# NVIDIA/audio-flamingo

Measured on AMD Instinct MI355X. Metric: audio-sec/s + decoder tokens/s, AF3-7B bf16 train, higher is better.
Workload: dtype bf16; 1 GPU; AF3 (AF-Whisper 32L + Qwen2.5-7B 28L, MLP projector) bf16 train step fwd+bwd+AdamW, 30 s clips, S=1024; micro_batch_per_gpu=8, global_batch=8, seq_len=1024, parallelism=dp1, activation_checkpointing=False

## Files before the change

audio-flamingo_amd/csrc/common.h:

```cpp
#pragma once
#include <hip/hip_runtime.h>
#include <stdint.h>
#include <stdio.h>
#include <stdarg.h>
#include <type_traits>
#include <utility>

typedef __bf16 bf16;
typedef __attribute__((ext_vector_type(2))) __bf16 bf16x2;
typedef __attribute__((ext_vector_type(4))) __bf16 bf16x4;
typedef __attribute__((ext_vector_type(8))) __bf16 bf16x8;
typedef __attribute__((ext_vector_type(2))) float f32x2;
typedef __attribute__((ext_vector_type(4))) float f32x4;
typedef __attribute__((ext_vector_type(16))) float f32x16;

#define AFK_OK 0
#define AFK_ERR_ARG (-1)
#define AFK_ERR_LAUNCH (-2)
#define AFK_ERR_UNSUPPORTED (-3)

int afk_set_error(int code, const char* fmt, ...);
void afk_count(int id);

#define AFK_REQUIRE(cond, ...)                                   \
// ... 110 lines not shown
    for (int i = 0; i < NW; ++i) r += scratch[i];
    return r;
}
template <int NW>
__device__ __forceinline__ float block_max(float v, float* scratch) {
    v = wave_max(v);
    const int lane = threadIdx.x & 63, w = threadIdx.x >> 6;
    __syncthreads();
    if (lane == 0) scratch[w] = v;
    __syncthreads();
    float r = scratch[0];
#pragma unroll
    for (int i = 1; i < NW; ++i) r = fmaxf(r, scratch[i]);
    return r;
}

__device__ __forceinline__ float sigmoid_f(float x) { return 1.f / (1.f + __expf(-x)); }
__device__ __forceinline__ float gelu_f(float x) { return 0.5f * x * (1.f + erff(x * 0.70710678118654752440f)); }
__device__ __forceinline__ float gelu_grad_f(float x) {
    const float cdf = 0.5f * (1.f + erff(x * 0.70710678118654752440f));
    const float pdf = 0.39894228040143267794f * __expf(-0.5f * x * x);
    return cdf + x * pdf;
}
```

audio-flamingo_amd/csrc/elementwise.hip:

```cpp
#include "common.h"
#include "../../include/afk.h"

namespace {

inline int ew_grid(int64_t n_items, int per_block) {
    int64_t g = afk_cdiv(n_items, per_block);
    if (g > 4096) g = 4096;
    if (g < 1) g = 1;
    return (int)g;
}

__global__ __launch_bounds__(256) void transpose_kernel(const bf16* __restrict__ in0, bf16* __restrict__ out0, int R, int C,
                                                        int Rpad, int64_t ld_in, int64_t ld_out, int nb2,
                                                        int64_t bs1_in, int64_t bs2_in, int64_t bs1_out, int64_t bs2_out,
                                                        int tiles_x, int tiles_y, int64_t ntiles) {
    __shared__ bf16 tile[64][66];
    const int t = threadIdx.x;
    for (int64_t tix = blockIdx.x; tix < ntiles; tix += gridDim.x) {
        const int bx = (int)(tix % tiles_x);
        const int by = (int)((tix / tiles_x) % tiles_y);
        const int b = (int)(tix / ((int64_t)tiles_x * tiles_y));
        const int b1 = b / nb2, b2 = b - b1 * nb2;
        const bf16* in = in0 + b1 * bs1_in + b2 * bs2_in;
        bf16* out = out0 + b1 * bs1_out + b2 * bs2_out;
        const int r0 = by * 64, c0 = bx * 64;
#pragma unroll
        for (int k = 0; k < 2; ++k) {
            const int idx = t + 256 * k;
            const int r = idx >> 3, ch = idx & 7;
            const int gr = r0 + r, gc = c0 + ch * 8;
            bf16x8 v;
            if (gr < R && gc + 7 < C) {
                v = *(const bf16x8*)(in + (int64_t)gr * ld_in + gc);
// ... 17 lines not shown
                if (gr + 7 < Rpad) {
                    *(bf16x8*)(out + (int64_t)gc * ld_out + gr) = v;
                } else {
                    for (int e = 0; e < 8 && gr + e < Rpad; ++e) out[(int64_t)gc * ld_out + gr + e] = v[e];
                }
            }
        }
        __syncthreads();
    }
}

__global__ __launch_bounds__(256) void gelu_bwd_kernel(const bf16* __restrict__ dy, const bf16* __restrict__ pre,
                                                       bf16* __restrict__ dx, int64_t nvec) {
    for (int64_t i = (int64_t)blockIdx.x * 256 + threadIdx.x; i < nvec; i += (int64_t)gridDim.x * 256) {
        const bf16x8 d = *(const bf16x8*)(dy + 8 * i);
        const bf16x8 p = *(const bf16x8*)(pre + 8 * i);
        bf16x8 o;
#pragma unroll
        for (int e = 0; e < 8; ++e) o[e] = (bf16)((float)d[e] * gelu_grad_f((float)p[e]));
        *(bf16x8*)(dx + 8 * i) = o;
    }
}

__global__ __launch_bounds__(256) void gelu_fwd_kernel(const bf16* __restrict__ x, bf16* __restrict__ y, int64_t nvec) {
    for (int64_t i = (int64_t)blockIdx.x * 256 + threadIdx.x; i < nvec; i += (int64_t)gridDim.x * 256) {
        const bf16x8 p = *(const bf16x8*)(x + 8 * i);
        bf16x8 o;
#pragma unroll
        for (int e = 0; e < 8; ++e) o[e] = (bf16)gelu_f((float)p[e]);
        *(bf16x8*)(y + 8 * i) = o;
    }
}


__global__ __launch_bounds__(256) void silu_mul_fwd_kernel(const bf16* __restrict__ gu, bf16* __restrict__ h, int64_t rows,
                                                           int I) {
    const int vpr = I >> 3;
    const int64_t total = rows * vpr;
    for (int64_t i = (int64_t)blockIdx.x * 256 + threadIdx.x; i < total; i += (int64_t)gridDim.x * 256) {
        const int64_t r = i / vpr;
        const int c = (int)(i - r * vpr) * 8;
        const bf16x8 g = *(const bf16x8*)(gu + r * 2 * I + c);
        const bf16x8 u = *(const bf16x8*)(gu + r * 2 * I + I + c);
        bf16x8 o;
#pragma unroll
        for (int e = 0; e < 8; ++e) {
            const float gf = (float)g[e];
            o[e] = (bf16)(rbf(gf * sigmoid_f(gf)) * (float)u[e]);
        }
        *(bf16x8*)(h + r * I + c) = o;
    }
}
// ... 683 lines not shown

#define ST ((hipStream_t)stream)

extern "C" int afk_transpose_bf16(const void* in, void* out, int R, int C, int Rpad, int64_t ld_in, int64_t ld_out, int nb1,
                                  int nb2, int64_t bs1_in, int64_t bs2_in, int64_t bs1_out, int64_t bs2_out, int max_blocks,
                                  void* stream) {
    AFK_REQUIRE(in && out && R > 0 && C > 0 && Rpad >= R && nb1 > 0 && nb2 > 0, "afk_transpose_bf16: bad args");
    AFK_REQUIRE(ld_in % 8 == 0 && ld_out % 8 == 0 && ((uintptr_t)in % 16 == 0) && ((uintptr_t)out % 16 == 0) &&
                    bs1_in % 8 == 0 && bs2_in % 8 == 0 && bs1_out % 8 == 0 && bs2_out % 8 == 0,
                "afk_transpose_bf16: 16-byte alignment required");
    const int tiles_x = (int)afk_cdiv(C, 64), tiles_y = (int)afk_cdiv(Rpad, 64);
    const int64_t ntiles = (int64_t)tiles_x * tiles_y * nb1 * nb2;
    int64_t grid = ntiles;
    if (grid > 65536) grid = 65536;
    if (max_blocks > 0 && grid > max_blocks) grid = max_blocks;
    hipLaunchKernelGGL(transpose_kernel, dim3((unsigned)grid), dim3(256), 0, ST, (const bf16*)in, (bf16*)out, R, C, Rpad, ld_in, ld_out,
                       nb2, bs1_in, bs2_in, bs1_out, bs2_out, tiles_x, tiles_y, ntiles);
    AFK_LAUNCH_CHECK("afk_transpose_bf16");
    return AFK_OK;
}

extern "C" int afk_gelu_fwd(const void* x, void* y, int64_t n, void* stream) {
    AFK_REQUIRE(x && y && n % 8 == 0, "afk_gelu_fwd: n must be a multiple of 8");
    hipLaunchKernelGGL(gelu_fwd_kernel, dim3(ew_grid(n / 8, 256)), dim3(256), 0, ST, (const bf16*)x, (bf16*)y, n / 8);
    AFK_LAUNCH_CHECK("afk_gelu_fwd");
    return AFK_OK;
}

extern "C" int afk_gelu_bwd(const void* dy, const void* pre, void* dx, int64_t n, void* stream) {
    AFK_REQUIRE(dy && pre && dx && n % 8 == 0, "afk_gelu_bwd: n must be a multiple of 8");
    hipLaunchKernelGGL(gelu_bwd_kernel, dim3(ew_grid(n / 8, 256)), dim3(256), 0, ST, (const bf16*)dy, (const bf16*)pre,
                       (bf16*)dx, n / 8);
    AFK_LAUNCH_CHECK("afk_gelu_bwd");
    return AFK_OK;
}

extern "C" int afk_silu_mul_fwd(const void* gu, void* h, int64_t rows, int I, void* stream) {
    AFK_REQUIRE(gu && h && I % 8 == 0 && rows > 0, "afk_silu_mul_fwd: bad args");
    hipLaunchKernelGGL(silu_mul_fwd_kernel, dim3(ew_grid(rows * (I / 8), 256)), dim3(256), 0, ST, (const bf16*)gu, (bf16*)h,
                       rows, I);
    AFK_LAUNCH_CHECK("afk_silu_mul_fwd");
    return AFK_OK;
}

extern "C" int afk_silu_mul_bwd(const void* gu, const void* dh, void* dgu, int64_t rows, int I, void* stream) {
    AFK_REQUIRE(gu && dh && dgu && I % 8 == 0 && rows > 0, "afk_silu_mul_bwd: bad args");
    hipLaunchKernelGGL(silu_mul_bwd_kernel, dim3(ew_grid(rows * (I / 8), 256)), dim3(256), 0, ST, (const bf16*)gu,
// ... 398 lines not shown
```

audio-flamingo_amd/csrc/gemm.hip:

```cpp
#include "gemm_common.h"
#include <vector>
#include <mutex>

namespace {

constexpr int BM = 128, BN = 128, BK = 64;
constexpr int ROWB = BK * 2;
constexpr int STAGE_BYTES = (BM + BN) * ROWB;
constexpr int NSTAGE = 2;

__global__ __launch_bounds__(256, 2) void gemm_nt_bf16_k128(GemmArgs p) {
    extern __shared__ __attribute__((aligned(16))) char smem[];
    const int tid = threadIdx.x;
    const int lane = tid & 63;
    const int wave = __builtin_amdgcn_readfirstlane(tid >> 6);
    const int wm = wave >> 1, wn = wave & 1;
    const int hi = lane >> 5, l31 = lane & 31;

    int tm, tn;
    gemm_tile_of_block(p, tm, tn);
    const int m0 = tm * BM, n0 = tn * BN;

    const bf16* a_src[4];
    const bf16* b_src[4];
// ... 314 lines not shown
        if (flags & (AFK_GEMM_RESIDUAL | AFK_GEMM_SWIGLU_BWD)) w = w && ldr % 8 == 0 && (uintptr_t)residual % 16 == 0;
        if (preact_out) w = w && (uintptr_t)preact_out % 16 == 0;
        p.wide = w && g_wide ? 1 : 0;
    }
    const int64_t tiles256 = afk_cdiv(M, 256) * afk_cdiv(N, 256);
    const bool use256 = !gemv && (trans_b || (flags & AFK_GEMM_SWIGLU_FWD) || (splits == 1 && (g_variant >= 2 || (g_variant == 0 && tiles256 >= 192))));
    if (rope && (!use256 || !p.wide || trans_a || trans_b || splits != 1))
        return afk_set_error(AFK_ERR_UNSUPPORTED, "afk_gemm_nt_bf16_rope: needs the 256 x 256 NT kernel (>= 192 tiles) in its 16-byte epilogue form; use "
                                                  "afk_gemm_nt_bf16 + afk_rope_inplace for this shape");
#ifdef AFK_PROBES
    static const int env_impl = [] {
        const char* e = getenv("AFK_GEMM256");
        return (e && e[0] == 'p' && e[1] == 'e') ? 13 : (e && e[0] == 'p') ? 2 : (e && e[0] == 'w') ? 3 : (e && e[0] == 'f') ? 10 : 0;
    }();
    const int impl256 = (flags & (AFK_GEMM_SWIGLU_FWD | AFK_GEMM_ROPE)) ? 2 : g_variant >= 2 ? (g_variant == 15 ? 2 : g_variant) : (env_impl ? env_impl : g_256_impl);
    const bool w4 = use256 && !trans_b && impl256 >= 3 && impl256 <= 9;
    const bool f8 = use256 && !trans_b && impl256 >= 10 && impl256 <= 12;
    const bool persist = use256 && !trans_b && impl256 == 13;
    const bool persist_q = use256 && !trans_b && impl256 == 14;
#endif
    if ((flags & AFK_GEMM_SWIGLU_FWD) && !p.wide)
        return afk_set_error(AFK_ERR_UNSUPPORTED, "afk_gemm_nt_bf16: SWIGLU_FWD needs the 16-byte epilogue form (aligned C / preact_out, ldc %% 8 == 0, "
                                                  "afk_gemm_set_variant bit 4 clear)");
    p.ntm = (int)afk_cdiv(M, use256 ? 256 : BM);
    p.ntn = (int)afk_cdiv(N, use256 ? 256 : BN);
    static bool attr_set = false;
    if (!attr_set) {
        hipFuncSetAttribute((const void*)gemm_nt_bf16_k128, hipFuncAttributeMaxDynamicSharedMemorySize, NSTAGE * STAGE_BYTES);
        attr_set = true;
    }
    hipStream_t st = (hipStream_t)stream;
    const int64_t nwg = (int64_t)p.ntm * p.ntn;
    AFK_REQUIRE(nwg < (1ll << 31), "afk_gemm_nt_bf16: grid too large");
    hipEvent_t e0 = nullptr, e1 = nullptr;
    bool prof = false;
    {
        std::lock_guard<std::mutex> lk(g_prof.mu);
        prof = g_prof.on;
        if (prof) {
            e0 = prof_next_event();
            e1 = prof_next_event();
            g_prof.flops += 2.0 * (double)M * (double)N * (double)K;
            g_prof.launches += 1;
            g_prof.recs.push_back({M, N, K, trans_b ? (trans_a ? 4 : 3) : (use256 ? 2 : 1)});
        }
    }
// ... 103 lines not shown
```

audio-flamingo_amd/csrc/gemm256.hip:

```cpp
#include "gemm_common.h"

namespace {

constexpr int BM = 256, BN = 256, BK = 64;
constexpr int ROWB = 128;
constexpr int OP_BYTES = 256 * ROWB;
constexpr int BUF_BYTES = 2 * OP_BYTES;
constexpr int LDS_BYTES = 2 * BUF_BYTES;

#define AFK_VMCNT(n) asm volatile("s_waitcnt vmcnt(" #n ")" ::: "memory")
#define AFK_LGKMCNT0() asm volatile("s_waitcnt lgkmcnt(0)" ::: "memory")
#define AFK_BARRIER()                         \
    do {                                      \
        __builtin_amdgcn_sched_barrier(0);    \
        __builtin_amdgcn_s_barrier();         \
        __builtin_amdgcn_sched_barrier(0);    \
    } while (0)

template <int EPI, int MF, bool OLDLOOP = false>
__global__ __launch_bounds__(512, 1) void gemm_nt_bf16_k256(GemmArgs p) {
    extern __shared__ __attribute__((aligned(16))) char smem[];
    const int tid = threadIdx.x;
    const int lane = tid & 63;
    const int wave = __builtin_amdgcn_readfirstlane(tid >> 6);
    const int wm = wave >> 2, wn = wave & 3;
    const int hi = lane >> 5, l31 = lane & 31;

    int tm, tn;
    gemm_tile_of_block(p, tm, tn);
    const int m0 = tm * BM, n0 = tn * BN;
    const int T = p.K / BK;
// ... 27 lines not shown
            __builtin_amdgcn_global_load_lds((gbl_void*)(xsrc[j] + koff), (lds_void*)(base + xdst[j]), 16, 0, 0);
    };
    auto issue_y = [&](int t) {
        char* base = smem + (t & 1) * BUF_BYTES;
        const int koff = t * BK;
#pragma unroll
        for (int j = 0; j < 2; ++j)
            __builtin_amdgcn_global_load_lds((gbl_void*)(ysrc[j] + koff), (lds_void*)(base + ydst[j]), 16, 0, 0);
    };
    __builtin_amdgcn_sched_barrier(0);
    issue_x(0);
    __builtin_amdgcn_sched_barrier(0);
#pragma unroll
    for (int j = 0; j < 2; ++j) {
        const int jj = wave + 8 * j;
        const int unit = jj < 8 ? 8 + jj : 16 + jj;
        const int rl = unit * 8 + lrow;
        const int chunk = pos ^ ((rl >> 1) & 7);
        const int r = min(m0 + rl, p.M - 1);
        ysrc[j] = p.A + (int64_t)r * p.lda + chunk * 8;
        ydst[j] = unit * 1024;
    }
    issue_y(0);
    if (T > 1) issue_x(1);
    __builtin_amdgcn_sched_barrier(0);

    int koffb[4];
#pragma unroll
    for (int x = 0; x < 4; ++x) koffb[x] = gemm_frag_rowoff<MF>(x) * ROWB + gemm_frag_koff<MF>(x, lane);
    const int a_row0 = (wm * 128 + gemm_frag_row<MF>(lane)) * ROWB;
    const int b_row0 = OP_BYTES + (wn * 64 + gemm_frag_row<MF>(lane)) * ROWB;

    GemmAcc<MF> acc;
    acc.zero();
#pragma unroll
    for (int x = 0; x < 4; ++x) afk_pin(koffb[x]);
    int a_row0_ = a_row0, b_row0_ = b_row0;
    afk_pin(a_row0_);
    afk_pin(b_row0_);
    acc.pin();

    if (T > 1) AFK_VMCNT(8);
    else AFK_VMCNT(2);
    AFK_BARRIER();
    if (wm == 1) AFK_BARRIER();

    bf16x8 bf[2][4], af[2][4];
    auto mfma_group = [&](auto acc0_, auto g_) {
        constexpr int ACC0 = decltype(acc0_)::value, g = decltype(g_)::value;
        if constexpr (MF == 32) {
#pragma unroll
            for (int i = 0; i < 2; ++i)
#pragma unroll
                for (int j = 0; j < 2; ++j) acc.mma(ACC0 + i, j, bf[j][g], af[i][g]);
        } else {
            constexpr int s = g >> 1, i = g & 1;
#pragma unroll
            for (int ih = 0; ih < 2; ++ih)
#pragma unroll
                for (int jt = 0; jt < 4; ++jt) acc.mma(2 * (ACC0 + i) + ih, jt, bf[jt >> 1][2 * (jt & 1) + s], af[i][2 * ih + s]);
        }
    };
    auto mfma_slot = [&](auto acc0_, auto q_) {
        constexpr int ACC0 = decltype(acc0_)::value, q = decltype(q_)::value;
        if constexpr (MF == 32) {
            constexpr int s = q >> 1, i = q & 1;
// ... 179 lines not shown
            const int64_t lbase = lanes ? (((int64_t)((m0 + wm * 128 + i * 32) % p.rope_S) >> 5) * 16 * 32 + l31) * 8 : 0;
#pragma unroll
            for (int j = 0; j < 2; ++j)
#pragma unroll
                for (int t = 0; t < 2; ++t) {
                    const int q = (i * 2 + j) * 2 + t;
                    const int cl = wn * 64 + j * 32 + 16 * t + 8 * hi;
                    b8 o = pc[q];
                    if (rot) {
                        const int d = cl & 127;
                        const b8 other = *(const b8*)(theirs + q * 1024);
                        const b8 c = lanes ? *(const b8*)(p.rope_cos_lanes + lbase + (d >> 3) * 256) : *(const b8*)(p.rope_cos + pr * 128 + d);
                        const b8 sn = lanes ? *(const b8*)(p.rope_sin_lanes + lbase + (d >> 3) * 256) : *(const b8*)(p.rope_sin + pr * 128 + d);
                        const float sg = (wn & 1) ? 1.f : -1.f;
#pragma unroll
                        for (int e = 0; e < 8; ++e)
                            o[e] = (bf16)(rbf_strict((float)pc[q][e] * (float)c[e]) + rbf_strict(sg * (float)other[e] * (float)sn[e]));
                    }
                    if (m < p.M) *(b8*)((bf16*)p.C + (int64_t)m * p.ldc + n0 + cl) = o;
                }
        }
        return;
    }
    if (AFK_GM_NOEPI(p)) return;
#pragma unroll
    for (int i = 0; i < 4; ++i)
#pragma unroll
        for (int j = 0; j < 2; ++j) gemm_store_block32<EPI, MF>(p, m0 + wm * 128 + i * 32, n0 + wn * 64 + j * 32, lane, acc.block(i, j));
}

}

#define AFK_EPI_LIST(X) X(0) X(AFK_GEMM_BIAS) X(AFK_GEMM_RESIDUAL) X(AFK_GEMM_BIAS | AFK_GEMM_RESIDUAL) X(AFK_GEMM_BIAS | AFK_GEMM_GELU) \
    X(AFK_GEMM_BIAS | AFK_GEMM_GELU | AFK_GEMM_RESIDUAL) X(AFK_GEMM_ACCUM) X(AFK_GEMM_SWIGLU_FWD) X(AFK_GEMM_SWIGLU_BWD) X(AFK_GEMM_ROPE) X(AFK_GEMM_ROPE | AFK_GEMM_BIAS) X(-1)

template <int MF, bool OLD = false>
static int launch_gemm256(const GemmArgs& p, hipStream_t st) {
    static bool attr_set = false;
    if (!attr_set) {
#define AFK_SET(F)                                                                                                                           \
    if (hipFuncSetAttribute((const void*)gemm_nt_bf16_k256<(F), MF, OLD>, hipFuncAttributeMaxDynamicSharedMemorySize, LDS_BYTES) != hipSuccess) \
        return afk_set_error(AFK_ERR_LAUNCH, "gemm256: cannot reserve %d bytes of LDS", LDS_BYTES);
        AFK_EPI_LIST(AFK_SET)
#undef AFK_SET
        attr_set = true;
    }
    const int64_t nwg = (int64_t)p.ntm * p.ntn;
    const int f = (p.wide && p.splits <= 1) ? p.flags : -1;
    switch (f) {
#define AFK_CASE(F)                                                                                              \
    case (F):                                                                                                    \
        if ((F) == -1) afk_count(AFK_CNT_GEMM_GENERIC);                                                          \
        hipLaunchKernelGGL((gemm_nt_bf16_k256<(F), MF, OLD>), dim3((unsigned)nwg), dim3(512), LDS_BYTES, st, p);      \
        break;
        AFK_EPI_LIST(AFK_CASE)
#undef AFK_CASE
        default:
            afk_count(AFK_CNT_GEMM_GENERIC);
            hipLaunchKernelGGL((gemm_nt_bf16_k256<-1, MF, OLD>), dim3((unsigned)nwg), dim3(512), LDS_BYTES, st, p);
    }
    return AFK_OK;
}

int afk_launch_gemm256(const GemmArgs& p, int mf, hipStream_t st) {
#ifdef AFK_PROBES
    if (AFK_GM_OLDLOOP(p)) return mf == 16 ? launch_gemm256<16, true>(p, st) : launch_gemm256<32, true>(p, st);
#endif
    if constexpr ((AFK_MFMA_SHAPES_NT & 2) != 0)
        if (mf == 16) return launch_gemm256<16>(p, st);
    if constexpr ((AFK_MFMA_SHAPES_NT & 1) != 0)
        if (mf == 32) return launch_gemm256<32>(p, st);
    return afk_set_error(AFK_ERR_UNSUPPORTED, "gemm256: the %s MFMA shape of the NT kernel is built under make PROBES=1 only", mf == 16 ? "16x16x32" : "32x32x16");
}
```

audio-flamingo_amd/csrc/gemm_common.h:

```cpp
#pragma once
#include "common.h"
#include "../../include/afk.h"

struct GemmArgs {
    const bf16* A;
    const bf16* B;
    void* C;
    void* C2;
    const bf16* bias;
    const bf16* R;
    int64_t lda, ldb, ldc, ldr;
    int M, N, K;
    int ntm, ntn;
    int flags;
    int res_mod;
    float alpha;
    int gm;
    int splits;
    float* ws;
    int wide;
    const bf16* rope_cos;
    const bf16* rope_sin;
    const int* rope_pos;
    int rope_S, rope_cols;
    const bf16* rope_cos_lanes;
    const bf16* rope_sin_lanes;
};

#ifdef AFK_PROBES
#define AFK_GM_NOEPI(p) (((p).gm & 0x40) != 0)
#define AFK_GM_RAW(p) (((p).gm & 0x80) != 0)
#define AFK_GM_OLDLOOP(p) (((p).gm & 0x100) != 0)
#else
#define AFK_GM_NOEPI(p) false
#define AFK_GM_RAW(p) false
#endif

typedef __attribute__((address_space(3))) void lds_void;
typedef const __attribute__((address_space(1))) void gbl_void;

__device__ __forceinline__ void gemm_tile_of(const GemmArgs& p, int bid, int nwg, int& tm, int& tn) {
    const int xcd = bid & 7, idx = bid >> 3, q = nwg >> 3, r = nwg & 7;
    const int swz = AFK_GM_RAW(p) ? bid : (xcd < r ? xcd * (q + 1) : r * (q + 1) + (xcd - r) * q) + idx;
    const int GM = (p.gm & 0x3f) > 0 ? (p.gm & 0x3f) : 4;
    const int per_group = GM * p.ntn;
    const int g = swz / per_group, rem = swz - g * per_group;
    const int first_m = g * GM;
    const int gsz = min(p.ntm - first_m, GM);
    tm = first_m + rem % gsz;
    tn = rem / gsz;
}
__device__ __forceinline__ void gemm_tile_of_block(const GemmArgs& p, int& tm, int& tn) { gemm_tile_of(p, blockIdx.x, gridDim.x, tm, tn); }

template <int W, int F = -1>
__device__ __forceinline__ void gemm_epilogue_store(const GemmArgs& p, int m, int n, float* v) {
    typedef __attribute__((ext_vector_type(W))) __bf16 bvec;
    typedef __attribute__((ext_vector_type(W))) float fvec;
    const int flags = F >= 0 ? F : p.flags;
#pragma unroll
    for (int e = 0; e < W; ++e) v[e] *= p.alpha;
    if (flags & AFK_GEMM_BIAS) {
        const bvec bv = *(const bvec*)(p.bias + n);
#pragma unroll
        for (int e = 0; e < W; ++e) v[e] += (float)bv[e];
    }
    if (flags & AFK_GEMM_GELU) {
#pragma unroll
        for (int e = 0; e < W; ++e) v[e] = rbf(v[e]);
        if (p.C2) {
            bvec pre;
#pragma unroll
            for (int e = 0; e < W; ++e) pre[e] = (bf16)v[e];
            *(bvec*)((bf16*)p.C2 + (int64_t)m * p.ldc + n) = pre;
        }
#pragma unroll
        for (int e = 0; e < W; ++e) v[e] = gelu_f(v[e]);
    }
    if (flags & AFK_GEMM_SWIGLU_BWD) {
        const bvec gv = *(const bvec*)(p.R + (int64_t)m * p.ldr + n);
        const bvec uv = *(const bvec*)(p.R + (int64_t)m * p.ldr + p.N + n);
        bvec og, ou;
#pragma unroll
        for (int e = 0; e < W; ++e) {
            const float gf = (float)gv[e], uf = (float)uv[e], df = rbf(v[e]);
            const float s = sigmoid_f(gf);
            og[e] = (bf16)(df * uf * (s * (1.f + gf * (1.f - s))));
            ou[e] = (bf16)(df * (gf * s));
        }
        bf16* cp = (bf16*)p.C + (int64_t)m * p.ldc + n;
        *(bvec*)cp = og;
        *(bvec*)(cp + p.N) = ou;
        return;
    }
    if (flags & AFK_GEMM_RESIDUAL) {
        const int rm = p.res_mod > 0 ? m % p.res_mod : m;
        const bvec rv = *(const bvec*)(p.R + (int64_t)rm * p.ldr + n);
#pragma unroll
        for (int e = 0; e < W; ++e) v[e] = rbf(v[e]) + (float)rv[e];
    }
// ... 93 lines not shown
__device__ __forceinline__ void gemm_lane_swap(float x, float y, float& lo, float& hi) {
    if constexpr (MF == 16) {
        const auto r = __builtin_amdgcn_permlane16_swap(__float_as_uint(x), __float_as_uint(y), false, false);
        lo = __uint_as_float(r[0]);
        hi = __uint_as_float(r[1]);
    } else {
        const auto r = __builtin_amdgcn_permlane32_swap(__float_as_uint(x), __float_as_uint(y), false, false);
        lo = __uint_as_float(r[0]);
        hi = __uint_as_float(r[1]);
    }
}
template <int MF>
__device__ __forceinline__ void gemm_quad_pos(int lane, int t, int h, int& row, int& col) {
    if (MF == 16) {
        row = 16 * h + (lane & 15);
        col = 16 * t + 4 * (lane >> 4);
    } else {
        row = lane & 31;
        col = 8 * (2 * t + h) + 4 * (lane >> 5);
    }
}

template <int F, int MF>
__device__ __forceinline__ void gemm_store_block32_body(const GemmArgs& p, int mb, int nb, int lane, const f32x16& b);
template <int MF>
static __device__ __noinline__ void gemm_store_block32_generic(const GemmArgs& p, int mb, int nb, int lane, f32x16 b) {
    gemm_store_block32_body<-1, MF>(p, mb, nb, lane, b);
}
template <int F = -1, int MF = 32>
__device__ __forceinline__ void gemm_store_block32(const GemmArgs& p, int mb, int nb, int lane, const f32x16& b) {
    if constexpr (F == -1) gemm_store_block32_generic<MF>(p, mb, nb, lane, b);
    else gemm_store_block32_body<F, MF>(p, mb, nb, lane, b);
}
template <int F, int MF>
__device__ __forceinline__ void gemm_store_block32_body(const GemmArgs& p, int mb, int nb, int lane, const f32x16& b) {
    if (F == -2 || (F == -1 && p.splits > 1)) {
#pragma unroll
        for (int t = 0; t < 2; ++t)
#pragma unroll
            for (int h = 0; h < 2; ++h) {
                int row, col;
                gemm_quad_pos<MF>(lane, t, h, row, col);
                const int m = mb + row, n = nb + col;
                if (m >= p.M || n >= p.N) continue;
                const f32x4 o = {b[8 * t + 4 * h], b[8 * t + 4 * h + 1], b[8 * t + 4 * h + 2], b[8 * t + 4 * h + 3]};
                *(f32x4*)(p.ws + ((int64_t)blockIdx.y * p.M + m) * p.N + n) = o;
            }
        return;
    }
    if constexpr (F == -2) return;
    if (F >= 0 || p.wide) {
        const int m = mb + (lane & 31);
#pragma unroll
        for (int t = 0; t < 2; ++t) {
            float v[8];
#pragma unroll
            for (int e = 0; e < 4; ++e) gemm_lane_swap<MF>(b[8 * t + e], b[8 * t + 4 + e], v[e], v[4 + e]);
            const int n = nb + 16 * t + 8 * (lane >> 5);
            if (m < p.M && n < p.N) gemm_epilogue_store<8, F>(p, m, n, v);
        }
        return;
    }
#pragma unroll
    for (int t = 0; t < 2; ++t)
#pragma unroll
        for (int h = 0; h < 2; ++h) {
            int row, col;
            gemm_quad_pos<MF>(lane, t, h, row, col);
            const int m = mb + row, n = nb + col;
            if (m >= p.M || n >= p.N) continue;
            float v[4] = {b[8 * t + 4 * h], b[8 * t + 4 * h + 1], b[8 * t + 4 * h + 2], b[8 * t + 4 * h + 3]};
            gemm_epilogue_store<4, F>(p, m, n, v);
        }
}

#ifdef AFK_PROBES
#define AFK_MFMA_SHAPES_NT 3
#define AFK_MFMA_SHAPES_NN 3
#define AFK_MFMA_SHAPES_TN 3
#else
#define AFK_MFMA_SHAPES_NT 2
#define AFK_MFMA_SHAPES_NN 1
// ... 10 lines not shown
```

audio-flamingo_amd/csrc/norm.hip:

```cpp
#include <algorithm>
#include "common.h"
#include "../../include/afk.h"

namespace {

constexpr int ROWS_PER_BLOCK = 4;
typedef __attribute__((ext_vector_type(4))) unsigned u32x4;

template <int VPL, bool RMS, int VW>
__global__ __launch_bounds__(256) void norm_fwd_kernel(const bf16* __restrict__ x, const bf16* __restrict__ w,
                                                       const bf16* __restrict__ b, bf16* __restrict__ y,
                                                       float* __restrict__ mean_out, float* __restrict__ rstd_out,
                                                       int64_t rows, int D, float eps) {
    const int lane = threadIdx.x & 63, wv = threadIdx.x >> 6;
    typedef __attribute__((ext_vector_type(VW))) __bf16 bvec;
    const int nvec = D / VW;
    const float invD = 1.f / (float)D;
    for (int64_t row = (int64_t)blockIdx.x * ROWS_PER_BLOCK + wv; row < rows; row += (int64_t)gridDim.x * ROWS_PER_BLOCK) {
        const bf16* xr = x + row * D;
        float v[VPL][VW];
        float s = 0.f, ss = 0.f;
#pragma unroll
        for (int i = 0; i < VPL; ++i) {
            const int vi = lane + 64 * i;
// ... 435 lines not shown
    return AFK_OK;
}

extern "C" int afk_layernorm_bwd(const void* x, const void* w, const void* dy, const float* mean, const float* rstd,
                                 void* dx, const void* dx_add, void* dw, void* db, int accumulate, float* workspace,
                                 int64_t rows, int D, void* stream) {
    AFK_REQUIRE(x && w && dy && mean && rstd && dx && dw && db && workspace, "afk_layernorm_bwd: null pointer");
    AFK_REQUIRE(D % 4 == 0 && D <= 4096 && (D <= 3584 || D % 8 == 0) && rows > 0, "afk_layernorm_bwd: unsupported D=%d", D);
    AFK_NORM_BWD_ALIGN("afk_layernorm_bwd");
    AFK_REQUIRE((uintptr_t)db % 8 == 0, "afk_layernorm_bwd: db must be 8-byte aligned");
    const bool cols = norm_bwd_use_cols(D);
    AFK_REQUIRE(cols || D <= 3584, "afk_layernorm_bwd: D=%d > 3584 is not served by the row-per-wave form (AFK_NORM_BWD=rows)", D);
    const int nb = std::min(cols ? norm_bwd_cols_blocks(rows, D, false) : norm_bwd_rowwave_blocks(rows), afk_norm_bwd_blocks(rows));
    hipStream_t st = (hipStream_t)stream;
    if (cols) launch_bwd_cols<false>(x, w, dy, mean, rstd, dx, dx_add, workspace, nb, rows, D, st);
    else launch_bwd<false>(x, w, dy, mean, rstd, dx, dx_add, workspace, nb, rows, D, st);
    hipLaunchKernelGGL(fold_partials_kernel, dim3((unsigned)afk_cdiv(D, 64), 2), dim3(256), 0, st, workspace, nb, D, 2 * D, (bf16*)dw, (bf16*)db,
                       accumulate);
    AFK_LAUNCH_CHECK("afk_layernorm_bwd");
    return AFK_OK;
}

namespace {
__global__ __launch_bounds__(256) void gelu_bwd_colsum_kernel(const bf16* __restrict__ dy, const bf16* __restrict__ pre, bf16* __restrict__ dx, int64_t rows, int C,
                                                              float* __restrict__ partials) {
    const int col = (blockIdx.y * 256 + threadIdx.x) * 8;
    if (col >= C) return;
    float pc[8];
#pragma unroll
    for (int e = 0; e < 8; ++e) pc[e] = 0.f;
    const int64_t step = gridDim.x;
    int64_t r = blockIdx.x;
    for (; r + 3 * step < rows; r += 4 * step) {
        bf16x8 d[4], p[4];
#pragma unroll
        for (int u = 0; u < 4; ++u) {
            d[u] = *(const bf16x8*)(dy + (r + u * step) * C + col);
            p[u] = *(const bf16x8*)(pre + (r + u * step) * C + col);
        }
#pragma unroll
        for (int u = 0; u < 4; ++u) {
            bf16x8 o;
#pragma unroll
            for (int e = 0; e < 8; ++e) {
                o[e] = (bf16)((float)d[u][e] * gelu_grad_f((float)p[u][e]));
                pc[e] += (float)o[e];
            }
            *(bf16x8*)(dx + (r + u * step) * C + col) = o;
        }
    }
    for (; r < rows; r += step) {
        const bf16x8 d = *(const bf16x8*)(dy + r * C + col), p = *(const bf16x8*)(pre + r * C + col);
        bf16x8 o;
#pragma unroll
        for (int e = 0; e < 8; ++e) {
            o[e] = (bf16)((float)d[e] * gelu_grad_f((float)p[e]));
            pc[e] += (float)o[e];
        }
        *(bf16x8*)(dx + r * C + col) = o;
    }
    float* outp = partials + (int64_t)blockIdx.x * C + col;
    *(f32x4*)(outp) = f32x4{pc[0], pc[1], pc[2], pc[3]};
    *(f32x4*)(outp + 4) = f32x4{pc[4], pc[5], pc[6], pc[7]};
}
}

extern "C" int afk_gelu_bwd_colsum_parts(int64_t rows) {
    static const int cap = [] { const char* e = getenv("AFK_GELU_CS_PARTS"); const int v = e ? atoi(e) : 0; return v > 0 ? v : 512; }();
    return (int)(rows < cap ? (rows < 1 ? 1 : rows) : cap);
}

extern "C" int afk_gelu_bwd_colsum(const void* dy, const void* pre, void* dx, int64_t rows, int C, void* colsum, int colsum_accumulate, float* workspace,
                                   void* stream) {
    AFK_REQUIRE(dy && pre && dx && colsum && workspace && rows > 0 && C > 0 && C % 8 == 0, "afk_gelu_bwd_colsum: bad arguments (C %% 8 == 0)");
    AFK_REQUIRE((uintptr_t)dy % 16 == 0 && (uintptr_t)pre % 16 == 0 && (uintptr_t)dx % 16 == 0 && (uintptr_t)workspace % 16 == 0 && (uintptr_t)colsum % 8 == 0,
                "afk_gelu_bwd_colsum: dy / pre / dx / workspace must be 16-byte aligned, colsum 8-byte aligned");
    hipStream_t st = (hipStream_t)stream;
    const int np = afk_gelu_bwd_colsum_parts(rows);
    hipLaunchKernelGGL(gelu_bwd_colsum_kernel, dim3((unsigned)np, (unsigned)afk_cdiv(C / 8, 256)), dim3(256), 0, st, (const bf16*)dy, (const bf16*)pre, (bf16*)dx, rows, C,
                       workspace);
    hipLaunchKernelGGL(fold_partials_kernel, dim3((unsigned)afk_cdiv(C, 64), 1), dim3(256), 0, st, workspace, np, C, C, (bf16*)colsum, (bf16*)nullptr, colsum_accumulate);
    AFK_LAUNCH_CHECK("afk_gelu_bwd_colsum");
    return AFK_OK;
}

extern "C" int afk_layernorm_bwd_colsum(const void* x, const void* w, const void* dy, const float* mean, const float* rstd, void* dx, const void* dx_add,
                                        void* dw, void* db, int accumulate, void* colsum, int colsum_accumulate, float* workspace, int64_t rows, int D,
                                        void* stream) {
    AFK_REQUIRE(x && w && dy && mean && rstd && dx && dx_add && dw && db && colsum && workspace, "afk_layernorm_bwd_colsum: null pointer");
    AFK_REQUIRE(D % 8 == 0 && D / 8 <= 512 && rows > 0, "afk_layernorm_bwd_colsum: unsupported D=%d (D %% 8 == 0, D <= 4096)", D);
    AFK_NORM_BWD_ALIGN("afk_layernorm_bwd_colsum");
    AFK_REQUIRE((uintptr_t)db % 8 == 0 && (uintptr_t)colsum % 8 == 0, "afk_layernorm_bwd_colsum: db / colsum must be 8-byte aligned");
    const int nb = std::min(norm_bwd_cols_blocks(rows, D, false), afk_norm_bwd_blocks(rows));
    hipStream_t st = (hipStream_t)stream;
    float* cs = workspace + (int64_t)afk_norm_bwd_blocks(rows) * 2 * D;
    const int nt = (int)afk_cdiv(D / 8, 64) * 64;
    hipLaunchKernelGGL((norm_bwd_cols_kernel<false, true, 2, true>), dim3(nb), dim3(nt), 0, st, (const bf16*)x, (const bf16*)w, (const bf16*)dy, mean, rstd,
                       (bf16*)dx, (const bf16*)dx_add, workspace, rows, D, cs);
    hipLaunchKernelGGL(fold_partials_kernel, dim3((unsigned)afk_cdiv(D, 64), 3), dim3(256), 0, st, workspace, nb, D, 2 * D, (bf16*)dw, (bf16*)db, accumulate,
                       (const float*)cs, D, (bf16*)colsum, colsum_accumulate);
    AFK_LAUNCH_CHECK("afk_layernorm_bwd_colsum");
    return AFK_OK;
}
// ... 19 lines not shown
```

audio-flamingo_amd/ops.py:

```python
from __future__ import annotations

import os

import torch

from . import _lib
from ._lib import AfkError

BF16 = torch.bfloat16

GEMM_BIAS, GEMM_GELU, GEMM_RESIDUAL, GEMM_OUT_F32, GEMM_ACCUM, GEMM_SWIGLU_BWD, GEMM_SWIGLU_FWD = 1, 2, 4, 8, 16, 32, 64


def _stream() -> int:
    return torch.cuda.current_stream().cuda_stream


def _p(t):
    return 0 if t is None else t.data_ptr()


def _chk(t: torch.Tensor, dtype=None, name="tensor"):
    if not t.is_cuda:
        raise AfkError(f"{name}: expected a HIP device tensor, got {t.device} (no CPU fallback in this package)")
# ... 1167 lines not shown
    if ws is None:
        ws = torch.empty(_lib.load().afk_sumsq_workspace_floats(), device=x.device, dtype=torch.float32)
    _lib.call("afk_sumsq_bf16", x.data_ptr(), x.numel(), _chk(acc, torch.float32).data_ptr(), _p(gate), ws.data_ptr(), _stream())
    return acc


def clip_coef_(sumsq, coef, *, max_norm, scale=1.0, norm_out=None):
    _lib.call("afk_clip_coef", _chk(sumsq, torch.float32).data_ptr(), sumsq.numel(), float(scale), float(max_norm), coef.data_ptr(), _p(norm_out), _stream())


def set_f32(dst, values):
    v = [float(x) for x in values] + [0.0] * (4 - len(values))
    _lib.call("afk_set_f32", _chk(dst, torch.float32).data_ptr(), len(values), v[0], v[1], v[2], v[3], _stream())


def gemm_set_variant(v: int):
    _lib.call("afk_gemm_set_variant", int(v))


def gemm_set_mfma(v: int):
    _lib.call("afk_gemm_set_mfma", int(v))


def gemm_mfma_shapes(form: str) -> tuple:
    mask = _lib.load().afk_gemm_mfma_shapes(("nt", "nn", "tn").index(form))
    return tuple(v for v in (1, 2) if mask >> (v - 1) & 1)


KERNEL_FAMILIES = ("gemm_nt128", "gemm_nt256", "gemm_nn256", "gemm_tn256", "gemm_splitk", "gemv", "attn2_fwd_d64", "attn2_fwd_d128",
                   "attn2_bwd_d64", "attn2_bwd_d128", "gqa_reduce", "xattn_fwd", "xattn_bwd", "attn1_fwd", "attn1_bwd", "gemm_generic_epilogue")


def kernel_counts(reset: bool = False) -> dict:
    import ctypes

    buf = (ctypes.c_int64 * len(KERNEL_FAMILIES))()
    _lib.call("afk_kernel_counts", ctypes.addressof(buf), len(KERNEL_FAMILIES))
    if reset:
        _lib.call("afk_kernel_counts_reset")
    return dict(zip(KERNEL_FAMILIES, list(buf)))


def prof_enable(on: bool):
    _lib.call("afk_prof_enable", int(on))


# ... 10 lines not shown
```

include/afk.h:

```cpp
#ifndef AFK_H
#define AFK_H
#include <stdint.h>
#ifdef __cplusplus
extern "C" {
#endif

int afk_version(void);
const char* afk_last_error(void);
const char* afk_build_id(void);
int afk_has_probes(void);

#define AFK_CNT_GEMM_NT128 0
#define AFK_CNT_GEMM_NT256 1
#define AFK_CNT_GEMM_NN256 2
#define AFK_CNT_GEMM_TN256 3
#define AFK_CNT_GEMM_SPLITK 4
#define AFK_CNT_GEMV 5
#define AFK_CNT_ATTN2_FWD_D64 6
#define AFK_CNT_ATTN2_FWD_D128 7
#define AFK_CNT_ATTN2_BWD_D64 8
#define AFK_CNT_ATTN2_BWD_D128 9
#define AFK_CNT_GQA_REDUCE 10
#define AFK_CNT_XATTN_FWD 11
#define AFK_CNT_XATTN_BWD 12
#define AFK_CNT_ATTN1_FWD 13
#define AFK_CNT_ATTN1_BWD 14
#define AFK_CNT_GEMM_GENERIC 15
#define AFK_CNT_MAX 16
int afk_kernel_counts(int64_t* host_out, int n);
int afk_kernel_counts_reset(void);

int afk_prof_enable(int on);
int afk_prof_reset(void);
int afk_prof_collect(double* host_total_ms, double* host_total_flops, int64_t* host_launches);
int afk_prof_dump(const char* host_path);

int afk_gemm_set_variant(int variant);
int afk_gemm_set_mfma(int v);
int afk_gemm_mfma_shapes(int form);
#define AFK_GEMM_BIAS 1
#define AFK_GEMM_GELU 2
#define AFK_GEMM_RESIDUAL 4
#define AFK_GEMM_OUT_F32 8
#define AFK_GEMM_ACCUM 16
#define AFK_GEMM_SWIGLU_BWD 32
#define AFK_GEMM_ROPE 128
#define AFK_GEMM_SWIGLU_FWD 64
int afk_gemm_nt_bf16(const void* A, int64_t lda, const void* B, int64_t ldb, void* C, int64_t ldc,
                     int M, int N, int K, const void* bias, const void* residual, int64_t ldr,
                     int res_mod, void* preact_out, float alpha, int flags, void* stream);
int afk_gemm_bf16(int trans_a, int trans_b, const void* A, int64_t lda, const void* B, int64_t ldb, void* C,
                  int64_t ldc, int M, int N, int K, const void* bias, const void* residual, int64_t ldr,
                  int res_mod, void* preact_out, float alpha, int flags, void* stream);
// ... 326 lines not shown
```

Measured before the change: 642.4 audio-s/s.

## Replace GELU erf evaluation with bf16-indexed LDS lookup tables

Builds per-device lookup tables of GELU and its gradient, indexed by bf16 bit pattern over a window of exponents, and stages them into LDS in the GEMM GELU epilogue, the standalone gelu forward kernel and the gelu backward colsum kernel. Vectors whose inputs all fall inside the window use a table read; the rest fall back to erf/exp evaluation. This targets the cost of transcendental math in epilogues and elementwise passes. In exchange it uses extra LDS (16 KB in the 256-tile GEMM, which can lower occupancy) and adds a table-load prologue to every block. The GEMM path indexes the table with the fp32 value truncated rather than rounded to bf16, so outputs may differ slightly from the computed GELU.

```diff
diff --git a/audio-flamingo_amd/csrc/act_lut.hip b/audio-flamingo_amd/csrc/act_lut.hip
--- /dev/null
+++ b/audio-flamingo_amd/csrc/act_lut.hip
@@ -0,0 +1,74 @@
+#include <mutex>
+
+#include "common.h"
+#include "../../include/afk.h"
+
+namespace {
+
+__global__ __launch_bounds__(256) void act_lut_fill_kernel(unsigned short* __restrict__ gelu, float* __restrict__ grad) {
+    const uint32_t i = blockIdx.x * 256 + threadIdx.x;
+    if (i >= AFK_LUT_PAD) return;
+    if (i >= AFK_LUT_N) {
+        gelu[i] = 0;
+        return;
+    }
+    const float x = afk_bf16_bits_to_f(afk_lut_bits_of(i));
+    gelu[i] = (unsigned short)afk_bf16_bits((bf16)gelu_f(x));
+    grad[i] = gelu_grad_f(x);
+}
+
+constexpr int MAX_DEV = 64;
+struct DevTables {
+    bool ready = false;
+    AfkActLut t = {nullptr, nullptr};
+};
+std::mutex g_mu;
+DevTables g_dev[MAX_DEV];
+constexpr int DEFAULT_MASK = AFK_LUT_ALL;
+int g_mask = DEFAULT_MASK;
+
+}
+
+extern "C" int afk_act_set_lut(int mask) {
+    AFK_REQUIRE(mask == -1 || (mask >= 0 && mask <= AFK_LUT_ALL), "afk_act_set_lut: mask %d (bits 0..2 = use sites, -1 = default)", mask);
+    g_mask = mask == -1 ? DEFAULT_MASK : mask;
+    return AFK_OK;
+}
+extern "C" int afk_act_get_lut(void) { return g_mask; }
+extern "C" int afk_act_lut_index(int bf16_bits) {
+    const uint32_t b = (uint32_t)bf16_bits & 0xffffu;
+    return afk_lut_in_window(b) ? (int)afk_lut_index(b) : -1;
+}
+
+bool afk_act_lut(int site, hipStream_t st, AfkActLut* out) {
+    if (!(g_mask & site)) return false;
+    int dev = 0;
+    if (hipGetDevice(&dev) != hipSuccess || dev < 0 || dev >= MAX_DEV) return false;
+    std::lock_guard<std::mutex> lk(g_mu);
+    DevTables& d = g_dev[dev];
+    if (!d.ready) {
+        hipStreamCaptureStatus cs = hipStreamCaptureStatusNone;
+        if (hipStreamIsCapturing(st, &cs) != hipSuccess || cs != hipStreamCaptureStatusNone) {
+            (void)hipGetLastError();
+            return false;
+        }
+        char* mem = nullptr;
+        const size_t b16 = AFK_LUT_PAD * sizeof(unsigned short);
+        if (hipMalloc((void**)&mem, b16 + AFK_LUT_N * sizeof(float)) != hipSuccess) {
+            (void)hipGetLastError();
+            return false;
+        }
+        unsigned short* ge = (unsigned short*)mem;
+        float* gr = (float*)(mem + b16);
+        hipLaunchKernelGGL(act_lut_fill_kernel, dim3(AFK_LUT_PAD / 256), dim3(256), 0, st, ge, gr);
+        if (hipGetLastError() != hipSuccess || hipStreamSynchronize(st) != hipSuccess) {
+            (void)hipGetLastError();
+            (void)hipFree(mem);
+            return false;
+        }
+        d.t = {ge, gr};
+        d.ready = true;
+    }
+    *out = d.t;
+    return true;
+}
diff --git a/audio-flamingo_amd/csrc/common.h b/audio-flamingo_amd/csrc/common.h
--- a/audio-flamingo_amd/csrc/common.h
+++ b/audio-flamingo_amd/csrc/common.h
@@ -156,3 +156,33 @@
     const float pdf = 0.39894228040143267794f * __expf(-0.5f * x * x);
     return cdf + x * pdf;
 }
+
+constexpr uint32_t AFK_LUT_EXP_LO = 111, AFK_LUT_EXPS = 24;
+constexpr uint32_t AFK_LUT_HALF = AFK_LUT_EXPS * 128;
+constexpr uint32_t AFK_LUT_N = 2 * AFK_LUT_HALF;
+constexpr uint32_t AFK_LUT_PAD = 8192;
+__host__ __device__ __forceinline__ uint32_t afk_lut_mag(uint32_t bits) { return (bits & 0x7fffu) - (AFK_LUT_EXP_LO << 7); }
+__host__ __device__ __forceinline__ bool afk_lut_in_window(uint32_t bits) { return afk_lut_mag(bits) < AFK_LUT_HALF; }
+__host__ __device__ __forceinline__ uint32_t afk_lut_index(uint32_t bits) { return afk_lut_mag(bits) + ((bits >> 15) & 1u) * AFK_LUT_HALF; }
+__host__ __device__ __forceinline__ uint32_t afk_lut_bits_of(uint32_t index) {
+    const uint32_t neg = index >= AFK_LUT_HALF ? 1u : 0u;
+    return (neg << 15) | (index - neg * AFK_LUT_HALF + (AFK_LUT_EXP_LO << 7));
+}
+__device__ __forceinline__ uint32_t afk_bf16_bits(bf16 x) { return __builtin_bit_cast(unsigned short, x); }
+__device__ __forceinline__ float afk_bf16_bits_to_f(uint32_t bits) { return __uint_as_float(bits << 16); }
+template <int W, typename V>
+__device__ __forceinline__ bool afk_lut_all_in(const V& x) {
+    uint32_t far = 0;
+#pragma unroll
+    for (int e = 0; e < W; ++e) far = max(far, afk_lut_mag(afk_bf16_bits(x[e])));
+    return far < AFK_LUT_HALF;
+}
+template <int NT>
+__device__ __forceinline__ void afk_lut_to_lds(void* lds, const void* tbl, int bytes) {
+    for (int i = threadIdx.x; i < bytes / 16; i += NT) ((uint4*)lds)[i] = ((const uint4*)tbl)[i];
+}
+struct AfkActLut {
+    const unsigned short* gelu;
+    const float* gelu_grad;
+};
+bool afk_act_lut(int site, hipStream_t st, AfkActLut* out);
diff --git a/audio-flamingo_amd/csrc/elementwise.hip b/audio-flamingo_amd/csrc/elementwise.hip
--- a/audio-flamingo_amd/csrc/elementwise.hip
+++ b/audio-flamingo_amd/csrc/elementwise.hip
@@ -1,3 +1,4 @@
+#include <algorithm>
 #include "common.h"
 #include "../../include/afk.h"
 
@@ -9,6 +10,8 @@
     if (g < 1) g = 1;
     return (int)g;
 }
+
+inline int ew_grid_lut(int64_t n_items, int per_block) { return std::min(ew_grid(n_items, per_block), 1536); }
 
 __global__ __launch_bounds__(256) void transpose_kernel(const bf16* __restrict__ in0, bf16* __restrict__ out0, int R, int C,
                                                         int Rpad, int64_t ld_in, int64_t ld_out, int nb2,
@@ -72,12 +75,23 @@
     }
 }
 
-__global__ __launch_bounds__(256) void gelu_fwd_kernel(const bf16* __restrict__ x, bf16* __restrict__ y, int64_t nvec) {
+template <bool LUT>
+__global__ __launch_bounds__(256) void gelu_fwd_kernel(const bf16* __restrict__ x, bf16* __restrict__ y, int64_t nvec, const unsigned short* __restrict__ tbl) {
+    __shared__ __attribute__((aligned(16))) unsigned short lut[LUT ? AFK_LUT_N : 8];
+    if constexpr (LUT) {
+        afk_lut_to_lds<256>(lut, tbl, AFK_LUT_N * 2);
+        __syncthreads();
+    }
     for (int64_t i = (int64_t)blockIdx.x * 256 + threadIdx.x; i < nvec; i += (int64_t)gridDim.x * 256) {
         const bf16x8 p = *(const bf16x8*)(x + 8 * i);
         bf16x8 o;
-#pragma unroll
-        for (int e = 0; e < 8; ++e) o[e] = (bf16)gelu_f((float)p[e]);
+        if (LUT && afk_lut_all_in<8>(p)) {
+#pragma unroll
+            for (int e = 0; e < 8; ++e) o[e] = __builtin_bit_cast(bf16, lut[afk_lut_index(afk_bf16_bits(p[e]))]);
+        } else {
+#pragma unroll
+            for (int e = 0; e < 8; ++e) o[e] = (bf16)gelu_f((float)p[e]);
+        }
         *(bf16x8*)(y + 8 * i) = o;
     }
 }
@@ -807,7 +821,11 @@
 
 extern "C" int afk_gelu_fwd(const void* x, void* y, int64_t n, void* stream) {
     AFK_REQUIRE(x && y && n % 8 == 0, "afk_gelu_fwd: n must be a multiple of 8");
-    hipLaunchKernelGGL(gelu_fwd_kernel, dim3(ew_grid(n / 8, 256)), dim3(256), 0, ST, (const bf16*)x, (bf16*)y, n / 8);
+    AfkActLut t;
+    if (afk_act_lut(AFK_LUT_GELU_FWD, ST, &t))
+        hipLaunchKernelGGL(gelu_fwd_kernel<true>, dim3(ew_grid_lut(n / 8, 256)), dim3(256), 0, ST, (const bf16*)x, (bf16*)y, n / 8, t.gelu);
+    else
+        hipLaunchKernelGGL(gelu_fwd_kernel<false>, dim3(ew_grid(n / 8, 256)), dim3(256), 0, ST, (const bf16*)x, (bf16*)y, n / 8, (const unsigned short*)nullptr);
     AFK_LAUNCH_CHECK("afk_gelu_fwd");
     return AFK_OK;
 }
diff --git a/audio-flamingo_amd/csrc/gemm.hip b/audio-flamingo_amd/csrc/gemm.hip
--- a/audio-flamingo_amd/csrc/gemm.hip
+++ b/audio-flamingo_amd/csrc/gemm.hip
@@ -360,6 +360,11 @@
     if ((flags & AFK_GEMM_SWIGLU_FWD) && !p.wide)
         return afk_set_error(AFK_ERR_UNSUPPORTED, "afk_gemm_nt_bf16: SWIGLU_FWD needs the 16-byte epilogue form (aligned C / preact_out, ldc %% 8 == 0, "
                                                   "afk_gemm_set_variant bit 4 clear)");
+    if (use256 && !trans_b && p.wide && splits == 1 && !rope) {
+        const bool gelu = flags == (AFK_GEMM_BIAS | AFK_GEMM_GELU) || flags == (AFK_GEMM_BIAS | AFK_GEMM_GELU | AFK_GEMM_RESIDUAL);
+        AfkActLut t;
+        if (gelu && afk_act_lut(AFK_LUT_GEMM_GELU, (hipStream_t)stream, &t)) p.lut = t.gelu;
+    }
     p.ntm = (int)afk_cdiv(M, use256 ? 256 : BM);
     p.ntn = (int)afk_cdiv(N, use256 ? 256 : BN);
     static bool attr_set = false;
diff --git a/audio-flamingo_amd/csrc/gemm256.hip b/audio-flamingo_amd/csrc/gemm256.hip
--- a/audio-flamingo_amd/csrc/gemm256.hip
+++ b/audio-flamingo_amd/csrc/gemm256.hip
@@ -7,6 +7,9 @@
 constexpr int OP_BYTES = 256 * ROWB;
 constexpr int BUF_BYTES = 2 * OP_BYTES;
 constexpr int LDS_BYTES = 2 * BUF_BYTES;
+constexpr int LUT_BYTES = AFK_LUT_PAD * 2;
+constexpr bool epi_has_lut(int epi) { return epi >= 0 && (epi & AFK_GEMM_GELU) != 0 && (epi & (AFK_GEMM_ROPE | AFK_GEMM_SWIGLU_FWD)) == 0; }
+constexpr int lds_bytes_of(int epi) { return LDS_BYTES + (epi_has_lut(epi) ? LUT_BYTES : 0); }
 
 #define AFK_VMCNT(n) asm volatile("s_waitcnt vmcnt(" #n ")" ::: "memory")
 #define AFK_LGKMCNT0() asm volatile("s_waitcnt lgkmcnt(0)" ::: "memory")
@@ -80,6 +83,18 @@
         ydst[j] = unit * 1024;
     }
     issue_y(0);
+    const bool use_lut = epi_has_lut(EPI) && p.lut != nullptr;
+    if constexpr (epi_has_lut(EPI)) {
+        __builtin_amdgcn_sched_barrier(0);
+        if (use_lut) {
+#pragma unroll
+            for (int j = 0; j < 2; ++j) {
+                const int piece = wave * 2 + j;
+                __builtin_amdgcn_global_load_lds((gbl_void*)((const char*)p.lut + piece * 1024 + lane * 16), (lds_void*)(smem + LDS_BYTES + piece * 1024), 16, 0, 0);
+            }
+        }
+        __builtin_amdgcn_sched_barrier(0);
+    }
     if (T > 1) issue_x(1);
     __builtin_amdgcn_sched_barrier(0);
 
@@ -98,8 +113,13 @@
     afk_pin(b_row0_);
     acc.pin();
 
-    if (T > 1) AFK_VMCNT(8);
-    else AFK_VMCNT(2);
+    if (use_lut) {
+        if (T > 1) AFK_VMCNT(10);
+        else AFK_VMCNT(4);
+    } else {
+        if (T > 1) AFK_VMCNT(8);
+        else AFK_VMCNT(2);
+    }
     AFK_BARRIER();
     if (wm == 1) AFK_BARRIER();
 
@@ -325,11 +345,12 @@
         }
         return;
     }
+    lds_u16* lut_lds = (lds_u16*)(lds_void*)(smem + LDS_BYTES);
     if (AFK_GM_NOEPI(p)) return;
 #pragma unroll
     for (int i = 0; i < 4; ++i)
 #pragma unroll
-        for (int j = 0; j < 2; ++j) gemm_store_block32<EPI, MF>(p, m0 + wm * 128 + i * 32, n0 + wn * 64 + j * 32, lane, acc.block(i, j));
+        for (int j = 0; j < 2; ++j) gemm_store_block32<EPI, MF>(p, m0 + wm * 128 + i * 32, n0 + wn * 64 + j * 32, lane, acc.block(i, j), lut_lds, use_lut);
 }
 
 }
@@ -342,8 +363,8 @@
     static bool attr_set = false;
     if (!attr_set) {
 #define AFK_SET(F)                                                                                                                           \
-    if (hipFuncSetAttribute((const void*)gemm_nt_bf16_k256<(F), MF, OLD>, hipFuncAttributeMaxDynamicSharedMemorySize, LDS_BYTES) != hipSuccess) \
-        return afk_set_error(AFK_ERR_LAUNCH, "gemm256: cannot reserve %d bytes of LDS", LDS_BYTES);
+    if (hipFuncSetAttribute((const void*)gemm_nt_bf16_k256<(F), MF, OLD>, hipFuncAttributeMaxDynamicSharedMemorySize, lds_bytes_of(F)) != hipSuccess) \
+        return afk_set_error(AFK_ERR_LAUNCH, "gemm256: cannot reserve %d bytes of LDS", lds_bytes_of(F));
         AFK_EPI_LIST(AFK_SET)
 #undef AFK_SET
         attr_set = true;
@@ -354,7 +375,7 @@
 #define AFK_CASE(F)                                                                                              \
     case (F):                                                                                                    \
         if ((F) == -1) afk_count(AFK_CNT_GEMM_GENERIC);                                                          \
-        hipLaunchKernelGGL((gemm_nt_bf16_k256<(F), MF, OLD>), dim3((unsigned)nwg), dim3(512), LDS_BYTES, st, p);      \
+        hipLaunchKernelGGL((gemm_nt_bf16_k256<(F), MF, OLD>), dim3((unsigned)nwg), dim3(512), lds_bytes_of(F), st, p); \
         break;
         AFK_EPI_LIST(AFK_CASE)
 #undef AFK_CASE
diff --git a/audio-flamingo_amd/csrc/gemm_common.h b/audio-flamingo_amd/csrc/gemm_common.h
--- a/audio-flamingo_amd/csrc/gemm_common.h
+++ b/audio-flamingo_amd/csrc/gemm_common.h
@@ -19,7 +19,10 @@
     int splits;
     float* ws;
     int wide;
-    const bf16* rope_cos;
+    union {
+        const bf16* rope_cos;
+        const unsigned short* lut;
+    };
     const bf16* rope_sin;
     const int* rope_pos;
     int rope_S, rope_cols;
@@ -38,6 +41,7 @@
 
 typedef __attribute__((address_space(3))) void lds_void;
 typedef const __attribute__((address_space(1))) void gbl_void;
+typedef const __attribute__((address_space(3))) unsigned short lds_u16;
 
 __device__ __forceinline__ void gemm_tile_of(const GemmArgs& p, int bid, int nwg, int& tm, int& tn) {
     const int xcd = bid & 7, idx = bid >> 3, q = nwg >> 3, r = nwg & 7;
@@ -53,7 +57,7 @@
 __device__ __forceinline__ void gemm_tile_of_block(const GemmArgs& p, int& tm, int& tn) { gemm_tile_of(p, blockIdx.x, gridDim.x, tm, tn); }
 
 template <int W, int F = -1>
-__device__ __forceinline__ void gemm_epilogue_store(const GemmArgs& p, int m, int n, float* v) {
+__device__ __forceinline__ void gemm_epilogue_store(const GemmArgs& p, int m, int n, float* v, lds_u16* lut = nullptr, bool use_lut = false) {
     typedef __attribute__((ext_vector_type(W))) __bf16 bvec;
     typedef __attribute__((ext_vector_type(W))) float fvec;
     const int flags = F >= 0 ? F : p.flags;
@@ -73,8 +77,20 @@
             for (int e = 0; e < W; ++e) pre[e] = (bf16)v[e];
             *(bvec*)((bf16*)p.C2 + (int64_t)m * p.ldc + n) = pre;
         }
-#pragma unroll
-        for (int e = 0; e < W; ++e) v[e] = gelu_f(v[e]);
+        bool in_table = false;
+        if (use_lut) {
+            uint32_t far = 0;
+#pragma unroll
+            for (int e = 0; e < W; ++e) far = max(far, afk_lut_mag(__float_as_uint(v[e]) >> 16));
+            in_table = far < AFK_LUT_HALF;
+        }
+        if (in_table) {
+#pragma unroll
+            for (int e = 0; e < W; ++e) v[e] = afk_bf16_bits_to_f(lut[afk_lut_index(__float_as_uint(v[e]) >> 16)]);
+        } else {
+#pragma unroll
+            for (int e = 0; e < W; ++e) v[e] = gelu_f(v[e]);
+        }
     }
     if (flags & AFK_GEMM_SWIGLU_BWD) {
         const bvec gv = *(const bvec*)(p.R + (int64_t)m * p.ldr + n);
@@ -214,18 +230,18 @@
 }
 
 template <int F, int MF>
-__device__ __forceinline__ void gemm_store_block32_body(const GemmArgs& p, int mb, int nb, int lane, const f32x16& b);
+__device__ __forceinline__ void gemm_store_block32_body(const GemmArgs& p, int mb, int nb, int lane, const f32x16& b, lds_u16* lut = nullptr, bool use_lut = false);
 template <int MF>
 static __device__ __noinline__ void gemm_store_block32_generic(const GemmArgs& p, int mb, int nb, int lane, f32x16 b) {
     gemm_store_block32_body<-1, MF>(p, mb, nb, lane, b);
 }
 template <int F = -1, int MF = 32>
-__device__ __forceinline__ void gemm_store_block32(const GemmArgs& p, int mb, int nb, int lane, const f32x16& b) {
+__device__ __forceinline__ void gemm_store_block32(const GemmArgs& p, int mb, int nb, int lane, const f32x16& b, lds_u16* lut = nullptr, bool use_lut = false) {
     if constexpr (F == -1) gemm_store_block32_generic<MF>(p, mb, nb, lane, b);
-    else gemm_store_block32_body<F, MF>(p, mb, nb, lane, b);
+    else gemm_store_block32_body<F, MF>(p, mb, nb, lane, b, lut, use_lut);
 }
 template <int F, int MF>
-__device__ __forceinline__ void gemm_store_block32_body(const GemmArgs& p, int mb, int nb, int lane, const f32x16& b) {
+__device__ __forceinline__ void gemm_store_block32_body(const GemmArgs& p, int mb, int nb, int lane, const f32x16& b, lds_u16* lut, bool use_lut) {
     if (F == -2 || (F == -1 && p.splits > 1)) {
 #pragma unroll
         for (int t = 0; t < 2; ++t)
@@ -249,7 +265,7 @@
 #pragma unroll
             for (int e = 0; e < 4; ++e) gemm_lane_swap<MF>(b[8 * t + e], b[8 * t + 4 + e], v[e], v[4 + e]);
             const int n = nb + 16 * t + 8 * (lane >> 5);
-            if (m < p.M && n < p.N) gemm_epilogue_store<8, F>(p, m, n, v);
+            if (m < p.M && n < p.N) gemm_epilogue_store<8, F>(p, m, n, v, lut, use_lut);
         }
         return;
     }
diff --git a/audio-flamingo_amd/csrc/norm.hip b/audio-flamingo_amd/csrc/norm.hip
--- a/audio-flamingo_amd/csrc/norm.hip
+++ b/audio-flamingo_amd/csrc/norm.hip
@@ -481,8 +481,31 @@
 }
 
 namespace {
+template <bool LUT>
 __global__ __launch_bounds__(256) void gelu_bwd_colsum_kernel(const bf16* __restrict__ dy, const bf16* __restrict__ pre, bf16* __restrict__ dx, int64_t rows, int C,
-                                                              float* __restrict__ partials) {
+                                                              float* __restrict__ partials, const float* __restrict__ tbl) {
+    __shared__ __attribute__((aligned(16))) float lut[LUT ? AFK_LUT_N : 4];
+    if constexpr (LUT) {
+        afk_lut_to_lds<256>(lut, tbl, AFK_LUT_N * 4);
+        __syncthreads();
+    }
+    auto grad8 = [&](const bf16x8& d, const bf16x8& p, float (&pc)[8]) {
+        bf16x8 o;
+        if (LUT && afk_lut_all_in<8>(p)) {
+#pragma unroll
+            for (int e = 0; e < 8; ++e) {
+                o[e] = (bf16)((float)d[e] * lut[afk_lut_index(afk_bf16_bits(p[e]))]);
+                pc[e] += (float)o[e];
+            }
+        } else {
+#pragma unroll
+            for (int e = 0; e < 8; ++e) {
+                o[e] = (bf16)((float)d[e] * gelu_grad_f((float)p[e]));
+                pc[e] += (float)o[e];
+            }
+        }
+        return o;
+    };
     const int col = (blockIdx.y * 256 + threadIdx.x) * 8;
     if (col >= C) return;
     float pc[8];
@@ -498,25 +521,11 @@
             p[u] = *(const bf16x8*)(pre + (r + u * step) * C + col);
         }
 #pragma unroll
-        for (int u = 0; u < 4; ++u) {
-            bf16x8 o;
-#pragma unroll
-            for (int e = 0; e < 8; ++e) {
-                o[e] = (bf16)((float)d[u][e] * gelu_grad_f((float)p[u][e]));
-                pc[e] += (float)o[e];
-            }
-            *(bf16x8*)(dx + (r + u * step) * C + col) = o;
-        }
+        for (int u = 0; u < 4; ++u) *(bf16x8*)(dx + (r + u * step) * C + col) = grad8(d[u], p[u], pc);
     }
     for (; r < rows; r += step) {
         const bf16x8 d = *(const bf16x8*)(dy + r * C + col), p = *(const bf16x8*)(pre + r * C + col);
-        bf16x8 o;
-#pragma unroll
-        for (int e = 0; e < 8; ++e) {
-            o[e] = (bf16)((float)d[e] * gelu_grad_f((float)p[e]));
-            pc[e] += (float)o[e];
-        }
-        *(bf16x8*)(dx + r * C + col) = o;
+        *(bf16x8*)(dx + r * C + col) = grad8(d, p, pc);
     }
     float* outp = partials + (int64_t)blockIdx.x * C + col;
     *(f32x4*)(outp) = f32x4{pc[0], pc[1], pc[2], pc[3]};
@@ -536,8 +545,12 @@
                 "afk_gelu_bwd_colsum: dy / pre / dx / workspace must be 16-byte aligned, colsum 8-byte aligned");
     hipStream_t st = (hipStream_t)stream;
     const int np = afk_gelu_bwd_colsum_parts(rows);
-    hipLaunchKernelGGL(gelu_bwd_colsum_kernel, dim3((unsigned)np, (unsigned)afk_cdiv(C / 8, 256)), dim3(256), 0, st, (const bf16*)dy, (const bf16*)pre, (bf16*)dx, rows, C,
-                       workspace);
+    const dim3 grid((unsigned)np, (unsigned)afk_cdiv(C / 8, 256));
+    AfkActLut t;
+    if (afk_act_lut(AFK_LUT_GELU_BWD_COLSUM, st, &t))
+        hipLaunchKernelGGL(gelu_bwd_colsum_kernel<true>, grid, dim3(256), 0, st, (const bf16*)dy, (const bf16*)pre, (bf16*)dx, rows, C, workspace, t.gelu_grad);
+    else
+        hipLaunchKernelGGL(gelu_bwd_colsum_kernel<false>, grid, dim3(256), 0, st, (const bf16*)dy, (const bf16*)pre, (bf16*)dx, rows, C, workspace, (const float*)nullptr);
     hipLaunchKernelGGL(fold_partials_kernel, dim3((unsigned)afk_cdiv(C, 64), 1), dim3(256), 0, st, workspace, np, C, C, (bf16*)colsum, (bf16*)nullptr, colsum_accumulate);
     AFK_LAUNCH_CHECK("afk_gelu_bwd_colsum");
     return AFK_OK;
diff --git a/audio-flamingo_amd/ops.py b/audio-flamingo_amd/ops.py
--- a/audio-flamingo_amd/ops.py
+++ b/audio-flamingo_amd/ops.py
@@ -1213,6 +1213,15 @@
     _lib.call("afk_gemm_set_mfma", int(v))
 
 
+ACT_LUT_SITES = {"gemm_gelu": 1, "gelu_fwd": 2, "gelu_bwd_colsum": 4}
+ACT_LUT_ALL = 7
+
+
+def act_set_lut(mask: int = -1) -> int:
+    _lib.call("afk_act_set_lut", int(mask))
+    return int(_lib.load().afk_act_get_lut())
+
+
 def gemm_mfma_shapes(form: str) -> tuple:
     mask = _lib.load().afk_gemm_mfma_shapes(("nt", "nn", "tn").index(form))
     return tuple(v for v in (1, 2) if mask >> (v - 1) & 1)
diff --git a/include/afk.h b/include/afk.h
--- a/include/afk.h
+++ b/include/afk.h
@@ -29,6 +29,14 @@
 #define AFK_CNT_MAX 16
 int afk_kernel_counts(int64_t* host_out, int n);
 int afk_kernel_counts_reset(void);
+
+#define AFK_LUT_GEMM_GELU 1
+#define AFK_LUT_GELU_FWD 2
+#define AFK_LUT_GELU_BWD_COLSUM 4
+#define AFK_LUT_ALL 7
+int afk_act_set_lut(int mask);
+int afk_act_get_lut(void);
+int afk_act_lut_index(int bf16_bits);
 
 int afk_prof_enable(int on);
 int afk_prof_reset(void);
```

After: 645.0 audio-s/s, median of 6. No clear change (+0.4%).
